# WhatAShot/Electrocardio-Panorama

Hardware: AMD Instinct MI355X
Metric: ECG-samples/sec (train step) (higher is better)
Workload: dtype f32 (conv products: fp32 operands split into fp16 hi+lo = 22-23 bits, block-scaled, 3 fp16 matrix products each, fp32 accumulate; fp32-class, not IEEE fp32)

## Files before the change

electrocardio_panorama_amd/_lib.py:

```python
import ctypes as C
import os

import torch

_HERE = os.path.dirname(os.path.abspath(__file__))
LIB_PATH = os.path.join(_HERE, "csrc", "libnefnet_hip.so")

NEF_OK = 0
_ERR = {-1: "NEF_E_SHAPE", -2: "NEF_E_NULL", -3: "NEF_E_WORKSPACE", -4: "NEF_E_UNSUPPORTED"}

p = C.c_void_p
i32 = C.c_int
i64 = C.c_int64
f32 = C.c_float
sz = C.c_size_t


class ConvArgs(C.Structure):
    _fields_ = [
        ("x", p), ("wp", p), ("y", p), ("bias", p), ("in_scale", p), ("res", p), ("gate", p), ("mask", p),
        ("x_bs", i64), ("x_gs", i64), ("y_bs", i64), ("y_gs", i64), ("sc_bs", i64), ("sc_gs", i64),
        ("res_bs", i64), ("res_gs", i64), ("gate_bs", i64), ("gate_gs", i64),
        ("B", i32), ("T", i32), ("G", i32), ("Cin_g", i32), ("Cout_g", i32), ("K", i32),
        ("relu", i32), ("gate_scale", f32), ("drop_scale", f32), ("drop_p", f32), ("rng_seed", C.c_uint64),
        ("pro_a", p), ("pro_b", p), ("pro_mode", i32), ("pro_Bp", i32), ("rng_seed_dev", p), ("wino", i32),
        ("stats", p),
        ("bnb_x", p), ("bnb_mean", p), ("bnb_invstd", p), ("bnb_a", p), ("bnb_b", p), ("bnb_slots", p), ("bnb_Bp", i32),
        ("bnb_up", i32), ("x_scale", f32), ("reserved0", i32), ("x_amax", p), ("x_amax_next", p), ("x_clamped", p),
        ("res_scale", p), ("rs_bs", i64), ("rs_gs", i64), ("gate_rowscale", p), ("gr_bs", i64), ("gr_gs", i64),
        ("stats_mode", i32), ("reserved1", i32),
    ]


class BwwArgs(C.Structure):
    _fields_ = [
        ("x", p), ("gy", p), ("gw", p), ("ws", p), ("in_scale", p), ("pro_a", p), ("pro_b", p),
        ("x_amax", p), ("gy_amax", p), ("x_amax_next", p), ("gy_amax_next", p), ("clamped", p), ("ws_bytes", sz),
        ("x_bs", i64), ("x_gs", i64), ("gy_bs", i64), ("gy_gs", i64), ("sc_bs", i64), ("sc_gs", i64),
        ("B", i32), ("T", i32), ("G", i32), ("Cin_g", i32), ("Cout_g", i32), ("K", i32),
        ("pro_mode", i32), ("pro_Bp", i32), ("form", i32), ("x_scale", f32), ("gy_scale", f32), ("reserved0", i32),
    ]


class BnBwdArgs(C.Structure):
    _fields_ = [
        ("g", p), ("gout", p), ("out", p), ("wout", p), ("x", p), ("mean", p), ("invstd", p), ("a", p), ("b", p),
        ("gx", p), ("ggamma", p), ("gbeta", p), ("gx_chan_sum", p), ("slots", p), ("ws", p), ("ws_bytes", sz),
        ("P", i32), ("Bp", i32), ("C", i32), ("L", i32), ("nslot", i32), ("form", i32), ("phase_major", i32), ("reserved0", i32),
    ]


class UpdateArgs(C.Structure):
    _fields_ = [
        ("p", p), ("g", p), ("buf", p), ("m", p), ("v", p), ("step", p), ("skip_if_positive", p), ("skipped", p), ("lr_dev", p),
        ("run_end", p), ("run_mul", p), ("n", i64), ("beta1", C.c_double), ("beta2", C.c_double),
        ("lr", f32), ("gscale", f32), ("mu", f32), ("eps", f32), ("weight_decay", f32),
        ("rule", i32), ("nesterov", i32), ("n_runs", i32),
    ]


class EmaArgs(C.Structure):
    _fields_ = [("ema", p), ("n_averaged", p), ("decay", C.c_double), ("warmup", i32), ("reserved0", i32)]


class PackDesc(C.Structure):
    _fields_ = [("w", p), ("wp", p), ("G", i32), ("Cog", i32), ("Cig", i32), ("K", i32), ("transpose_flip", i32),
                ("wino", i32), ("src_mode", i32), ("src_Cr", i32)]


SIGNATURES = {
    "nef_abi_version": (i32, []),
    "nef_debug_spin_us": (i32, [f32, i32, p]),
    "nef_stem_fwd": (i32, [p, p, p, i32, i32, i32, p]),
    "nef_stem_bwd_ws_bytes": (sz, [i32]),
    "nef_stem_bwd_weight": (i32, [p, p, p, p, p, sz, i32, i32, i32, p]),
    "nef_pack_weight": (i32, [p, p, i32, i32, i32, i32, i32, p]),
    "nef_pack_weight_wino": (i32, [p, p, i32, i32, i32, i32, i32, p]),
    "nef_pack_weight_wino4": (i32, [p, p, i32, i32, i32, i32, i32, p]),
    "nef_pack_weights": (i32, [C.POINTER(PackDesc), i32, p]),
    "nef_pack_weight_h2": (i32, [p, p, i32, i32, i32, i32, i32, p]),
    "nef_pack_weight_h2_bytes": (sz, [i32, i32, i32, i32, i32]),
    "nef_conv_fwd": (i32, [C.POINTER(ConvArgs), p]),
# ... 18 lines not shown
    "nef_theta_encode": (i32, [p, p, i32, p]),
    "nef_chscale_fwd": (i32, [p, p, i64, p, i32, i32, i32, p]),
    "nef_chscale_bwd": (i32, [p, p, p, i64, p, p, i32, i32, i32, i32, p]),
    "nef_gate": (i32, [p, p, p, f32, i64, p]),
    "nef_add": (i32, [p, p, p, i64, p]),
    "nef_roi_align_fwd": (i32, [p, p, p, i32, i32, i32, i32, i32, p]),
    "nef_roi_align_bwd": (i32, [p, p, p, i32, i32, i32, i32, i32, p]),
    "nef_window_crop": (i32, [p, i64, i64, p, i32, i32, i32, i32, i32, i32, p]),
    "nef_window_scatter": (i32, [p, p, i64, i64, i32, i32, i32, i32, i32, i32, p]),
    "nef_roi_unpool_fwd": (i32, [p, p, p, p, i32, i32, i32, p]),
    "nef_roi_unpool_bwd": (i32, [p, p, p, i32, i32, i32, p]),
    "nef_roi_segment_table": (i32, [p, p, p, i32, p]),
    "nef_lead_mean": (i32, [p, p, p, i32, i32, i32, p]),
    "nef_mix_fwd": (i32, [p, p, p, p, p, i32, i32, i32, i32, i32, p, p]),
    "nef_mix_bwd": (i32, [p, p, p, p, p, p, p, p, i32, i32, i32, i32, i32, p, i32, i32, i32, p]),
    "nef_mix_fwd_shared": (i32, [p, p, p, p, p, i32, i32, i32, i32, i32, p, p]),
    "nef_lead_mean_mix_shared": (i32, [p, p, p, p, p, i32, i32, i32, i32, i32, p, p]),
    "nef_pass_combine_fwd": (i32, [p, p, p, i32, i32, i32, p]),
    "nef_pass_combine_bwd": (i32, [p, p, i32, i32, i32, p]),
    "nef_pass_combine_stats_ws_bytes": (sz, [i32, i32]),
    "nef_pass_combine_fwd_stats": (i32, [p, p, p, p, p, p, p, p, p, p, p, p, sz, i32, i32, i32, f32, f32, p, p]),
    "nef_upsample2_fwd": (i32, [p, p, i64, i32, p]),
    "nef_upsample2_bwd": (i32, [p, p, i64, i32, p]),
    "nef_bn_ws_bytes": (sz, [i32, i32]),
    "nef_bn_train_stats": (i32, [p, p, p, p, p, p, p, p, p, p, sz, i32, i32, i32, i32, f32, f32, p, p]),
    "nef_conv_stats_slots": (i32, [i32, i32]),
    "nef_bn_stats_from_slots": (i32, [p, i32, p, p, p, p, p, p, p, p, p, sz, i32, i32, i32, i32, f32, f32, p, p]),
    "nef_bn_eval_affine": (i32, [p, p, p, p, p, p, i32, f32, p]),
    "nef_fold_bn": (i32, [p, p, p, p, p, p, i32, i32, p]),
    "nef_affine_relu_fwd": (i32, [p, p, p, p, i32, i32, i32, i32, p]),
    "nef_bn_bwd_ws_bytes": (sz, [C.POINTER(BnBwdArgs)]),
    "nef_bn_relu_bwd": (i32, [C.POINTER(BnBwdArgs), p]),
    "nef_bn_bwd_args_bytes": (sz, []),
    "nef_outconv_fwd": (i32, [p, p, p, i32, p, p, p, i32, i32, i32, p]),
    "nef_outconv_bwd_weight": (i32, [p, p, p, p, p, i32, p, p, p, sz, i32, i32, i32, p]),
    "nef_outconv_bwd_data": (i32, [p, p, p, p, i32, i32, i32, p]),
    "nef_outconv_bwd_weight_ws_bytes": (sz, [i32]),
    "nef_loss_ws_bytes": (sz, []),
    "nef_loss_fwd": (i32, [p, p, p, p, p, p, sz, i64, f32, f32, f32, i32, i32, p]),
    "nef_loss_bwd": (i32, [p, p, p, p, p, p, p, p, i64, f32, f32, f32, i32, i32, p]),
    "nef_loss_noise_fwd": (i32, [p, p, p, p, p, p, p, sz, i64, f32, f32, f32, i32, i32, p]),
    "nef_loss_noise_bwd": (i32, [p, p, p, p, p, p, p, p, p, i64, f32, f32, f32, i32, i32, p]),
    "nef_sgd_momentum": (i32, [p, p, p, i64, f32, f32, f32, i32, p, p, p, p]),
    "nef_adam": (i32, [p, p, p, p, i64, f32, C.c_double, C.c_double, f32, f32, f32, p, p, p, p, p]),
    "nef_update": (i32, [C.POINTER(UpdateArgs), p]),
    "nef_update_args_bytes": (sz, []),
    "nef_update_ema": (i32, [C.POINTER(UpdateArgs), C.POINTER(EmaArgs), p]),
    "nef_ema_args_bytes": (sz, []),
    "nef_grad_clip_ws_bytes": (sz, []),
    "nef_grad_clip": (i32, [p, i64, f32, f32, p, p, p, sz, p]),
    "nef_h2_taint": (i32, [p, p, p, p]),
    "nef_amax_roll": (i32, [p, p, i32, f32, f32, i32, p]),
    "nef_step_words": (i32, [p, p, i32, i32, i64, p]),
    "nef_flatten": (i32, [C.POINTER(p), C.POINTER(i64), i32, p, p]),
    "nef_regroup_halves": (i32, [p, p, i32, i32, i32, i32, p]),
    "nef_slots_to_rows": (i32, [p, i32, p, i32, i32, p]),
    "nef_poly_weights": (i32, [p, p, i32, i32, i32, p]),
    "nef_poly_fwd_edge": (i32, [p, p, p, i32, i32, i32, i32, i32, p, p, i32, p, i32, p, p]),
    "nef_poly_wgrad_fold_ws_bytes": (sz, [i32, i32, i32, i32]),
    "nef_poly_wgrad_fold": (i32, [p, p, p, p, p, sz, i32, i32, i32, i32, i32, p]),
    "nef_poly_bwd_edge": (i32, [p, p, p, i32, i32, i32, i32, i32, p, p, p, p, p, i32, p, i32, i32, p]),
    "nef_view_metrics": (i32, [p, p, p, p, p, i32, i32, i32, p]),
    "nef_pano_h_from_f32": (i32, [p, p, i32, i32, i32, p]),
    "nef_pano_h_pack_weight": (i32, [p, p, i32, i32, p]),
    "nef_pano_h_conv": (i32, [p, p, p, p, p, i32, i32, i32, i32, i32, i32, i32, i64, i64, p]),
    "nef_pano_h_conv_pair": (i32, [p, p, p, p, p, p, p, i32, i32, i32, i32, i64, i64, p]),
    "nef_pano_h_conv_outconv": (i32, [p, p, p, p, p, p, i32, i32, i32, i64, i64, p]),
    "nef_pano_h_conv_tail": (i32, [p, p, p, p, p, p, p, p, i32, i32, i32, i64, i64, p]),
    "nef_pano_h_outconv": (i32, [p, p, p, p, i32, i32, i32, i64, i64, p]),
}

_lib = None


class NefLibraryError(RuntimeError):
    pass


def load():
    global _lib
    if _lib is not None:
        return _lib
    if not os.path.exists(LIB_PATH):
        raise NefLibraryError(
            f"{LIB_PATH} not found: the HIP extension is required (no CPU fallback). "
            "Build it with `python -m electrocardio_panorama_amd.csrc.build`.")
    lib = C.CDLL(LIB_PATH)
    for name, (res, args) in SIGNATURES.items():
        fn = getattr(lib, name)
        fn.restype = res
        fn.argtypes = args
    for name, size, mirror in (("nef_conv_args", lib.nef_conv_args_bytes(), ConvArgs),
                               ("nef_bww_args", lib.nef_bww_args_bytes(), BwwArgs),
                               ("nef_bn_bwd_args", lib.nef_bn_bwd_args_bytes(), BnBwdArgs),
                               ("nef_update_args", lib.nef_update_args_bytes(), UpdateArgs),
                               ("nef_ema_args", lib.nef_ema_args_bytes(), EmaArgs)):
        if size != C.sizeof(mirror):
            raise NefLibraryError(f"{LIB_PATH}: {name} is {size} bytes, the binding mirrors {C.sizeof(mirror)}; rebuild with "
                                  "`python -m electrocardio_panorama_amd.csrc.build`")
    _lib = lib
    return lib


def check(rc, what=""):
    if rc == NEF_OK:
        return
    if rc < 0:
        raise NefLibraryError(f"{what}: {_ERR.get(rc, rc)}")
    raise NefLibraryError(f"{what}: hipError_t {rc}")
```

electrocardio_panorama_amd/csrc/elementwise.hip:

```cpp
#include "nef_common.h"

namespace {

__global__ void chscale_fwd_kernel(const float* __restrict__ x, const float* __restrict__ s, int64_t s_bs,
                                   float* __restrict__ y, int B, int C, int T) {
    const int64_t rows = (int64_t)B * C;
    const int wave = threadIdx.x >> 6, lane = threadIdx.x & 63;
    for (int64_t row = (int64_t)blockIdx.x * 4 + wave; row < rows; row += (int64_t)gridDim.x * 4) {
        const int b = (int)(row / C), c = (int)(row % C);
        const float f = s[(int64_t)b * s_bs + c];
        const float* xr = x + row * T;
        float* yr = y + row * T;
        for (int t = lane; t < T; t += 64) yr[t] = xr[t] * f;
    }
}

__global__ void chscale_bwd_kernel(const float* __restrict__ gy, const float* __restrict__ x,
                                   const float* __restrict__ s, int64_t s_bs, float* __restrict__ gx,
                                   float* __restrict__ gs, int B, int C, int T, int relu_x) {
    const int64_t rows = (int64_t)B * C;
    const int wave = threadIdx.x >> 6, lane = threadIdx.x & 63;
    for (int64_t row = (int64_t)blockIdx.x * 4 + wave; row < rows; row += (int64_t)gridDim.x * 4) {
        const int b = (int)(row / C), c = (int)(row % C);
        const float f = s[(int64_t)b * s_bs + c];
// ... 658 lines not shown
                s2 += (double)g * (double)((xv - mf) * is);
            }
        }
    }
    s1 = nef_block_sum_d(s1, sm);
    s2 = nef_block_sum_d(s2, sm);
    if (threadIdx.x == 0) {
        part[((int64_t)(p * C + c) * BN_SPLIT + sp) * 2] = s1;
        part[((int64_t)(p * C + c) * BN_SPLIT + sp) * 2 + 1] = s2;
    }
}

__global__ void bn_bwd_final(const double* __restrict__ part, float* __restrict__ coef, float* __restrict__ ggamma,
                             float* __restrict__ gbeta, int P, int Bp, int C, int L, int nsplit = BN_SPLIT) {
    const int c = blockIdx.x * blockDim.x + threadIdx.x;
    if (c >= C) return;
    const double n = (double)Bp * (double)L;
    double g1 = 0.0, g2 = 0.0;
    for (int p = 0; p < P; ++p) {
        double s1 = 0.0, s2 = 0.0;
        for (int sp = 0; sp < nsplit; ++sp) {
            s1 += part[((int64_t)(p * C + c) * nsplit + sp) * 2];
            s2 += part[((int64_t)(p * C + c) * nsplit + sp) * 2 + 1];
        }
        coef[(p * C + c) * 2] = (float)(s1 / n);
        coef[(p * C + c) * 2 + 1] = (float)(s2 / n);
        g1 += s1;
        g2 += s2;
    }
    gbeta[c] = (float)g1;
    ggamma[c] = (float)g2;
}

__global__ void bn_bwd_apply(const float* __restrict__ gy, const float* __restrict__ x, const float* __restrict__ mean,
                             const float* __restrict__ invstd, const float* __restrict__ a, const float* __restrict__ b,
                             const float* __restrict__ coef, float* __restrict__ gx, double* __restrict__ rowsum, int P,
                             int Bp, int C, int L) {
    const int64_t rows = (int64_t)P * Bp * C;
    const int wave = threadIdx.x >> 6, lane = threadIdx.x & 63;
    for (int64_t row = (int64_t)blockIdx.x * 4 + wave; row < rows; row += (int64_t)gridDim.x * 4) {
        const int c = (int)(row % C);
        const int p = (int)(row / ((int64_t)Bp * C));
        const int pc = p * C + c;
        const float mf = mean[pc], is = invstd[pc], af = a[pc], bf = b[pc];
        const float k1 = coef[pc * 2], k2 = coef[pc * 2 + 1];
        const float* xr = x + row * L;
        const float* gr = gy + row * L;
        float* gxr = gx + row * L;
        double rs = 0.0;
        if ((L & 3) == 0) {
            const int L4 = L >> 2;
#pragma unroll 2
            for (int t = lane; t < L4; t += 64) {
                const nef_f32x4 xv = ((const nef_f32x4*)xr)[t], gv = ((const nef_f32x4*)gr)[t];
                nef_f32x4 o;
#pragma unroll
                for (int e = 0; e < 4; ++e) {
                    const float g = fmaf(xv[e], af, bf) > 0.f ? gv[e] : 0.f;
                    o[e] = af * (g - k1 - (xv[e] - mf) * is * k2);
                    rs += (double)o[e];
                }
                ((nef_f32x4*)gxr)[t] = o;
            }
        } else {
            for (int t = lane; t < L; t += 64) {
                const float xv = xr[t];
// ... 1446 lines not shown
        if (form == 1)
            hipLaunchKernelGGL(bn_bwd_partial<1>, grid, dim3(256), 0, NEF_ST, g, a.x, a.mean, a.invstd, a.a, a.b, part, P, Bp, C, L,
                               a.wout);
        else if (form == 2)
            hipLaunchKernelGGL(bn_bwd_partial<2>, grid, dim3(256), 0, NEF_ST, g, a.x, a.mean, a.invstd, a.a, a.b, part, P, Bp, C, L,
                               (const float*)nullptr);
        else
            hipLaunchKernelGGL(bn_bwd_partial<0>, grid, dim3(256), 0, NEF_ST, g, a.x, a.mean, a.invstd, a.a, a.b, part, P, Bp, C, L,
                               (const float*)nullptr);
        hipLaunchKernelGGL(bn_bwd_final, dim3((C + 63) / 64), dim3(64), 0, NEF_ST, (const double*)part, coef, a.ggamma, a.gbeta, P, Bp, C,
                           L, BN_SPLIT);
    }
    const dim3 grid((unsigned)rows);
    if (form == 3)
        hipLaunchKernelGGL(bn_bwd_apply_combine3, dim3((unsigned)(Bp * C)), dim3(256), 0, NEF_ST, g, a.x, a.mean, a.invstd, a.a, a.b,
                           (const float*)coef, a.gx, rowsum, Bp, C, L, deint);
    else if (form == 2)
        hipLaunchKernelGGL(bn_bwd_apply_rows<2>, grid, dim3(256), 0, NEF_ST, g, a.x, a.mean, a.invstd, a.a, a.b, (const float*)coef, a.gx,
                           rowsum, Bp, C, L >> 2, (const float*)nullptr);
    else if (form == 1)
        hipLaunchKernelGGL(bn_bwd_apply_rows<1>, grid, dim3(256), 0, NEF_ST, g, a.x, a.mean, a.invstd, a.a, a.b, (const float*)coef, a.gx,
                           rowsum, Bp, C, L >> 2, a.wout);
    else if (by_rows)
        hipLaunchKernelGGL(bn_bwd_apply_rows<0>, grid, dim3(256), 0, NEF_ST, g, a.x, a.mean, a.invstd, a.a, a.b, (const float*)coef, a.gx,
                           rowsum, Bp, C, L >> 2, (const float*)nullptr, deint);
    else
        hipLaunchKernelGGL(bn_bwd_apply, dim3(nef_stream_grid(rows, 4)), dim3(256), 0, NEF_ST, g, a.x, a.mean, a.invstd, a.a, a.b,
                           (const float*)coef, a.gx, rowsum, P, Bp, C, L);
    if (a.gx_chan_sum)
        hipLaunchKernelGGL(rowsum_to_channel, dim3(C), dim3(256), 0, NEF_ST, (const double*)rowsum, a.gx_chan_sum, P * Bp, C);
    return nef_launch_status();
}

int nef_outconv_fwd(const float* x, const float* a, const float* b, int Bp, const float* w, const float* bias,
                    float* out, int N, int C, int L, nef_stream_t stream) {
    NEF_ENTER();
    NEF_REQUIRE(x && w && bias && out, NEF_E_NULL);
    NEF_REQUIRE((a == nullptr) == (b == nullptr), NEF_E_NULL);
    NEF_REQUIRE(N > 0 && C > 0 && C <= OC_MAXC && L > 0 && (!a || Bp > 0), NEF_E_SHAPE);
    if ((L & 3) == 0) {
        const int tiles = (L + 1023) / 1024;
        hipLaunchKernelGGL(outconv_fwd_kernel<true>, dim3((unsigned)((int64_t)N * tiles)), dim3(256), 0, NEF_ST, x, w, bias,
                           out, N, C, L, tiles, a, b, a ? Bp : 1);
        return nef_launch_status();
    }
    const int tiles = (L + 255) / 256;
    hipLaunchKernelGGL(outconv_fwd_kernel<false>, dim3((unsigned)((int64_t)N * tiles)), dim3(256), 0, NEF_ST, x, w, bias,
                       out, N, C, L, tiles, a, b, a ? Bp : 1);
    return nef_launch_status();
}

int nef_outconv_bwd_data(const float* gout, const float* out, const float* w, float* gx, int N, int C, int L,
                         nef_stream_t stream) {
    NEF_ENTER();
    NEF_REQUIRE(gout && out && w && gx, NEF_E_NULL);
    NEF_REQUIRE(N > 0 && C > 0 && C <= OC_MAXC && L > 0, NEF_E_SHAPE);
    const int tiles = (L + 255) / 256;
    hipLaunchKernelGGL(outconv_bwd_data_kernel, dim3((unsigned)((int64_t)N * tiles)), dim3(256), 0, NEF_ST, gout, out,
                       w, gx, N, C, L, tiles);
    return nef_launch_status();
}

size_t nef_outconv_bwd_weight_ws_bytes(int C) { return (size_t)OC_BLOCKS * (C + 1) * 3 * sizeof(double); }

int nef_outconv_bwd_weight(const float* gout, const float* out, const float* x, const float* a, const float* b, int Bp,
                           float* gw, float* gb, void* ws, size_t ws_bytes, int N, int C, int L, nef_stream_t stream) {
// ... 254 lines not shown
```

electrocardio_panorama_amd/engine.py:

```python
import os

import torch
from . import _env

from . import ops
from .ops import GV

N_SEG, ROI_BINS = 7, 16
DROP_P = 0.2
BN_EPS, BN_MOM = 1e-5, 0.1


DROPOUT_SITES = ("W_encoder.layer1.0", "W_encoder.layer1.1", "W_encoder.layer1.2", "w_conv.0", "z1_conv.0",
                 "z2_conv1.0", "z2_conv2.0", "z2_conv2.2")


class DropCfg:

    def __init__(self, training, p=DROP_P, masks=None, seed=0, seed_dev=None):
        self.seed_dev = seed_dev
        self.on = bool(training) and p > 0.0
        self.p = p if self.on else 0.0
        self.scale = 1.0 / (1.0 - p) if self.on else 1.0
        self.masks = masks
# ... 107 lines not shown
    xv, h, y, prefix, K, Cog, res_conv, dscale = saved[:8]
    in_scale = saved[8] if len(saved) > 8 else None
    side = side or ops._Inline()
    G, Cig = xv.G, xv.Cg
    g2 = gy if pre_gated else ops.gate(gy, y)
    g2v, hv = GV.dense(g2, G), GV.dense(h, G)
    grads[prefix + ".conv2.weight"] = side.run(lambda: ops.conv_bwd_weight(hv, g2v, K, site=P[prefix + ".conv2.weight"].data_ptr()), h, g2)
    gc1 = ops.conv(g2v, ops.pack_weight(P[prefix + ".conv2.weight"], G, flip=True, T=xv.T, f4=_bwd_f4(K)), Cog, K, gate=hv,
                   gate_scale=dscale, role="conv_bwd_data")
    gc1v = GV.dense(gc1, G)
    grads[prefix + ".conv1.weight"] = side.run(lambda: ops.conv_bwd_weight(xv, gc1v, K, in_scale=in_scale, site=P[prefix + ".conv1.weight"].data_ptr()), xv.t, gc1)
    if res_conv:
        grads[prefix + ".residual_conv.weight"] = side.run(lambda: ops.conv_bwd_weight(xv, g2v, 1, site=P[prefix + ".residual_conv.weight"].data_ptr()), xv.t, g2)
        grads[prefix + ".residual_conv.bias"] = side.run(lambda: ops.chan_sum(g2), g2)
        gres = ops.conv(g2v, ops.pack_weight(P[prefix + ".residual_conv.weight"], G, flip=True, T=xv.T), Cig, 1,
                        role="conv_bwd_data")
        resv = GV.dense(gres, G)
    else:
        resv = g2v
    wp1f = ops.pack_weight(P[prefix + ".conv1.weight"], G, flip=True, T=xv.T, f4=_bwd_f4(K))
    if in_scale is not None and scale_bwd and int(getattr(wp1f, "nef_wino", 0)) == 3 and out is None:
        slots = ops.conv_stats_buffer(wp1f, xv.B, G, Cig, xv.T, xv.t.device)
        if slots is not None:
            gx = ops.conv(gc1v, wp1f, Cig, K, res=resv, gate=xv, gate_scale=1.0, gate_rowscale=in_scale, stats=slots, stats_mode=1,
                          role="conv_bwd_data")
            return gx, ops.slots_to_rows(slots, xv.B)
    return ops.conv(gc1v, wp1f, Cig, K, res=resv,
                    out=out, gate=xv if gate_input else None, gate_scale=1.0, role="conv_bwd_data")


_DEC = (("decoder.1", "0", "1", 128), ("decoder.1", "3", "4", 128), ("decoder.3", "0", "1", 64),
        ("decoder.3", "3", "4", 64))


_HALVES = "decoder.1.double_conv.0.weight#halves"


def _regroup_halves(w, P=None):
    if P is not None:
        hit = P.get(_HALVES)
        if hit is not None and hit[1] is w and hit[2] == w._version:
            return hit[0]
    wg = ops.regroup_halves(w)
    if P is not None:
        P[_HALVES] = (wg, w, w._version)
    return wg


def _ungroup_halves(w2):
    return ops.regroup_halves(w2, inverse=True)


def _fusable(D, passes):
    return 2 * D.shape[2] >= 128


def _decoder_fwd_unfused(D, P, Bf, passes, training, save):
    x = D
    saved = []
    for li, (blk, cv, bn, cout) in enumerate(_DEC):
        if li in (0, 2):
            x = ops.upsample2_fwd(x)
        wname, bname, pre = f"{blk}.double_conv.{cv}.weight", f"{blk}.double_conv.{cv}.bias", f"{blk}.double_conv.{bn}"
        c = ops.conv(GV.dense(x, 1), ops.pack_weight(P[wname], 1, T=x.shape[2], f4=True), cout, 3, bias=P[bname])
        if training:
            mean, invstd, a, b = ops.bn_train_stats(c, P[pre + ".weight"], P[pre + ".bias"], Bf[pre + ".running_mean"],
# ... 56 lines not shown
        else:
            wp = ops.pack_weight(P[wname], 1, T=T_out, f4=True)
            slots = ops.conv_stats_buffer(wp, N, 1, cout, T_out, D.device) if training else None
            c = ops.conv(GV.dense(x_in, 1), wp, cout, 3, bias=P[bname], pro=pro, stats=slots)
            if slots is not None:
                stats = ops.bn_stats_from_slots(slots, P[pre + ".weight"], P[pre + ".bias"], Bf[pre + ".running_mean"],
                                                Bf[pre + ".running_var"], passes, N, T_out, BN_EPS, BN_MOM,
                                                nbt=Bf[pre + ".num_batches_tracked"])
        if stats is not None:
            mean, invstd, a, b = stats
            Bp = N // passes
        elif training:
            mean, invstd, a, b = ops.bn_train_stats(c, P[pre + ".weight"], P[pre + ".bias"], Bf[pre + ".running_mean"],
                                                    Bf[pre + ".running_var"], passes, BN_EPS, BN_MOM, nbt=Bf[pre + ".num_batches_tracked"])
            Bp = N // passes
        else:
            a, b = ops.bn_eval_affine(P[pre + ".weight"], P[pre + ".bias"], Bf[pre + ".running_mean"],
                                      Bf[pre + ".running_var"], BN_EPS)
            mean = invstd = None
            Bp = N
        if save:
            saved.append((x_in, c, mean, invstd, a, b, pro, up_after, xedge))
        x, pro_in = c, (a, b, Bp)
    out = ops.outconv_fwd(x, P["decoder.4.weight"], P["decoder.4.bias"], pro=pro_in)
    return out, (saved, x, out, passes, pro_in, shared_B)


def decoder_bwd(dsaved, g_out, P, grads, side=None):
    saved, c4, out, passes, pro4 = dsaved[:5]
    shared_B = dsaved[5] if len(dsaved) > 5 else None
    side = side or ops._Inline()
    if len(dsaved) > 5:
        ops.pack_many(_decoder_pack_requests(P, c4.shape[2] // 4, True))
    grads["decoder.4.weight"], grads["decoder.4.bias"] = side.run(
        lambda: ops.outconv_bwd_weight(g_out, out, c4, pro=pro4), g_out, out, c4)
    fuse_last = c4.shape[2] % 4 == 0
    g_is_up = False
    g = None if fuse_last else ops.outconv_bwd_data(g_out, out, P["decoder.4.weight"], c4.shape[1])
    g_slots = None
    poly_first = False
    for li in (3, 2, 1, 0):
        blk, cv, bn, cout = _DEC[li]
        x, c, mean, invstd, a, b, pro, up_after = saved[li][:8]
        xedge = saved[li][8] if len(saved[li]) > 8 else None
        sh0 = li == 0 and shared_B is not None
        Cog_, Cig_ = c.shape[1], x.shape[1] // (2 if sh0 else 1)
        poly_b = bool(up_after and pro[0] & 2 and (not sh0 or pro[0] == 2) and ops.poly_bwd_ok(2 if sh0 else 1, Cog_, Cig_, c.shape[2]))
        pm = bool(poly_b and xedge is not None and ops.poly_w_ok((2 if sh0 else 1) * (shared_B if sh0 else c.shape[0]), 2 if sh0 else 1, Cog_, Cig_, c.shape[2]))
        wname, bname, pre = f"{blk}.double_conv.{cv}.weight", f"{blk}.double_conv.{cv}.bias", f"{blk}.double_conv.{bn}"
        pm0_done = False
        if li == 3 and fuse_last:
            gc, gg, gbeta, gbias = ops.bn_relu_bwd_outconv(g_out, out, P["decoder.4.weight"], c, mean, invstd, a, b, passes)
        elif li == 0 and shared_B is not None and not g_is_up:
            gc, gg, gbeta, gbias = ops.bn_relu_bwd_combine3(g, c, mean, invstd, a, b, slots=g_slots, phase_major=pm)
            pm0_done = pm
        elif g_is_up:
            gc, gg, gbeta, gbias = ops.bn_relu_bwd_up(g, c, mean, invstd, a, b, passes, slots=g_slots)
        else:
            gc, gg, gbeta, gbias = ops.bn_relu_bwd(g, c, P[pre + ".weight"], mean, invstd, a, b, passes,
                                                   with_chan_sum=True, slots=g_slots, phase_major=pm and not sh0)
            pm0_done = pm and not sh0
        grads[pre + ".weight"], grads[pre + ".bias"], grads[bname] = gg, gbeta, gbias
        pm = pm and pm0_done
        if li == 0 and shared_B is not None:
            gp2 = gc if gc.shape[0] == 2 * shared_B else ops.pass_combine_bwd(gc)
            gpv, xv = GV.dense(gp2, 2), GV.dense(x, 2)
            if pm:
                grads[wname] = side.run(lambda: _ungroup_halves(ops.conv_bwd_weight_poly(xv, gp2, Cog_, pro, xedge, site=P[wname].data_ptr())), x, gp2, xedge)
            else:
                grads[wname] = side.run(lambda: _ungroup_halves(ops.conv_bwd_weight(xv, gpv, 3, pro=pro, site=P[wname].data_ptr())), x, gp2)
            if poly_b:
                g = ops.conv_bwd_data_poly(gpv, _regroup_halves(P[wname], P), x.shape[1] // 2, site=P[wname].data_ptr(), phase_major=pm)
                poly_first = True
            else:
                g = ops.conv(gpv, ops.pack_weight(_regroup_halves(P[wname], P), 2, flip=True, T=gp2.shape[2], f4=True, site=P[wname].data_ptr()), x.shape[1] // 2, 3,
                             role="conv_bwd_data")
        else:
            gcv, xv = GV.dense(gc, 1), GV.dense(x, 1)
            if pm:
                grads[wname] = side.run(lambda: ops.conv_bwd_weight_poly(xv, gc, Cog_, pro, xedge, site=P[wname].data_ptr()), x, gc, xedge)
            else:
                grads[wname] = side.run(lambda: ops.conv_bwd_weight(xv, gcv, 3, pro=pro, site=P[wname].data_ptr()), x, gc)
            if poly_b:
                bnb = None
# ... 324 lines not shown
```

electrocardio_panorama_amd/ops.py:

```python
import ctypes as C
import contextlib
import itertools
import os

import torch
from . import _env

from . import _lib

N_SEG, ROI_BINS = 7, 16


def _p(t):
    return None if t is None else t.data_ptr()


def _stream():
    return torch.cuda.current_stream().cuda_stream


def _chk(t, dtype=torch.float32):
    assert t.is_cuda and t.dtype == dtype and t.is_contiguous(), (t.device, t.dtype, t.is_contiguous())
    return t

# ... 1249 lines not shown

def bn_relu_bwd(gy, x, gamma, mean, invstd, a, b, P, with_chan_sum=False, slots=None, phase_major=False):
    _chk(gy), _chk(x)
    N, Ct, Ln = x.shape
    gx = torch.empty(N, 2 * Ct, Ln // 2, device=x.device, dtype=torch.float32) if phase_major else torch.empty_like(x)
    r = _bn_bwd(0, "bn_relu_bwd", (gy, x, gx), x, mean, invstd, a, b, P, gx, with_chan_sum, slots, phase_major, g=gy)
    return r if with_chan_sum else r[:3]


def bn_relu_bwd_combine3(gy, x, mean, invstd, a, b, slots=None, phase_major=False):
    _chk(gy), _chk(x)
    N, Ct, Ln = x.shape
    Bp = N // 3
    gP2 = torch.empty((2 * Bp, 4 * Ct, Ln // 2) if phase_major else (2 * Bp, 2 * Ct, Ln), device=x.device, dtype=torch.float32)
    return _bn_bwd(3, "bn_relu_bwd_combine3", (gy, x, gP2), x, mean, invstd, a, b, 3, gP2, slots=slots, phase_major=phase_major,
                   g=gy)


def bn_relu_bwd_up(gu, x, mean, invstd, a, b, P, slots=None):
    _chk(gu), _chk(x)
    N, Ct, Ln = x.shape
    assert gu.shape == (N, Ct, 2 * Ln)
    gx = torch.empty_like(x)
    return _bn_bwd(2, "bn_relu_bwd_up", (gu, x, gx), x, mean, invstd, a, b, P, gx, slots=slots, g=gu)


def bn_relu_bwd_outconv(gout, out, wout, x, mean, invstd, a, b, P):
    _chk(gout), _chk(out), _chk(x)
    gx = torch.empty_like(x)
    return _bn_bwd(1, "bn_relu_bwd_outconv", (gout, out, x, gout, out, x, gx), x, mean, invstd, a, b, P, gx, gout=gout, out=out,
                   wout=wout)


def outconv_fwd(x, w, bias, pro=None):
    L = _lib.load()
    _chk(x), _chk(w), _chk(bias)
    N, Ct, Ln = x.shape
    out = torch.empty(N, 1, Ln, device=x.device, dtype=torch.float32)
    a, b, Bp = pro if pro is not None else (None, None, 1)
    ev = _hbm("outconv_fwd", x, out)
    _lib.check(L.nef_outconv_fwd(_p(x), _p(a), _p(b), Bp, _p(w), _p(bias), _p(out), N, Ct, Ln, _stream()), "nef_outconv_fwd")
    _done(ev)
    return out


def outconv_bwd_data(gout, out, w, Ct):
    L = _lib.load()
    _chk(gout), _chk(out)
    N, Ln = out.shape[0], out.shape[-1]
    gx = torch.empty(N, Ct, Ln, device=out.device, dtype=torch.float32)
    _lib.check(L.nef_outconv_bwd_data(_p(gout), _p(out), _p(w), _p(gx), N, Ct, Ln, _stream()), "nef_outconv_bwd_data")
    return gx


def outconv_bwd_weight(gout, out, x, pro=None):
    L = _lib.load()
    _chk(gout), _chk(out), _chk(x)
    N, Ct, Ln = x.shape
    gw = torch.empty(1, Ct, 3, device=x.device, dtype=torch.float32)
    gb = torch.empty(1, device=x.device, dtype=torch.float32)
    n = L.nef_outconv_bwd_weight_ws_bytes(Ct)
    ws = workspace(n, x.device)
    a, b, Bp = pro if pro is not None else (None, None, 1)
    ev = _hbm("outconv_bwd_weight", gout, out, x)
    _lib.check(L.nef_outconv_bwd_weight(_p(gout), _p(out), _p(x), _p(a), _p(b), Bp, _p(gw), _p(gb), _p(ws), n, N, Ct, Ln,
                                        _stream()), "nef_outconv_bwd_weight")
# ... 258 lines not shown
```

include/nefnet_hip.h:

```cpp
#ifndef NEFNET_HIP_H
#define NEFNET_HIP_H

#include <stddef.h>
#include <stdint.h>

#ifdef __cplusplus
extern "C" {
#endif

#define NEF_OK 0
#define NEF_E_SHAPE (-1)
#define NEF_E_NULL (-2)
#define NEF_E_WORKSPACE (-3)
#define NEF_E_UNSUPPORTED (-4)

#define NEF_N_SEG 7
#define NEF_ROI_BINS 16

typedef void* nef_stream_t;

int nef_abi_version(void);

int nef_debug_spin_us(float us, int wgs, nef_stream_t stream);

// ... 187 lines not shown
                       float* a, float* b, int C, float eps, nef_stream_t stream);
int nef_fold_bn(const float* w, const float* bias, const float* a, const float* b, float* w_out, float* bias_out,
                int Cout, int inner, nef_stream_t stream);
int nef_affine_relu_fwd(const float* x, const float* a, const float* b, float* y, int P, int Bp, int C, int L,
                        nef_stream_t stream);
typedef struct nef_bn_bwd_args {
    const float* g;
    const float* gout;
    const float* out;
    const float* wout;
    const float* x;
    const float* mean;
    const float* invstd;
    const float* a;
    const float* b;
    float* gx;
    float* ggamma;
    float* gbeta;
    float* gx_chan_sum;
    const float* slots;
    void* ws;
    size_t ws_bytes;
    int32_t P, Bp, C, L;
    int32_t nslot;
    int32_t form;
    int32_t phase_major;
    int32_t reserved0;
} nef_bn_bwd_args;

int nef_bn_relu_bwd(const nef_bn_bwd_args* a, nef_stream_t stream);
size_t nef_bn_bwd_ws_bytes(const nef_bn_bwd_args* a);
size_t nef_bn_bwd_args_bytes(void);

int nef_outconv_fwd(const float* x, const float* a, const float* b, int Bp, const float* w, const float* bias,
                    float* out, int N, int C, int L, nef_stream_t stream);
int nef_outconv_bwd_weight(const float* gout, const float* out, const float* x, const float* a, const float* b, int Bp,
                           float* gw, float* gb, void* ws, size_t ws_bytes, int N, int C, int L, nef_stream_t stream);
int nef_outconv_bwd_data(const float* gout, const float* out, const float* w, float* gx, int N, int C, int L,
                         nef_stream_t stream);
size_t nef_outconv_bwd_weight_ws_bytes(int C);

size_t nef_loss_ws_bytes(void);
int nef_loss_fwd(const float* pred, const float* pred_p, const float* pred_l, const float* target, float* losses,
                 void* ws, size_t ws_bytes, int64_t n, float f0, float f1, float f2, int reg_l2, int use_mask,
                 nef_stream_t stream);
int nef_loss_bwd(const float* pred, const float* pred_p, const float* pred_l, const float* target,
                 const float* gscale , float* g_pred, float* g_p, float* g_l, int64_t n, float f0,
                 float f1, float f2, int reg_l2, int use_mask, nef_stream_t stream);
int nef_loss_noise_fwd(const float* pred, const float* pred_p, const float* pred_l, const float* target,
                       const float* noise, float* losses, void* ws, size_t ws_bytes, int64_t n, float f0, float f1, float f2,
                       int reg_l2, int use_mask, nef_stream_t stream);
int nef_loss_noise_bwd(const float* pred, const float* pred_p, const float* pred_l, const float* target,
                       const float* noise, const float* gscale , float* g_pred, float* g_p, float* g_l,
                       int64_t n, float f0, float f1, float f2, int reg_l2, int use_mask, nef_stream_t stream);

int nef_sgd_momentum(float* p, const float* g, float* buf, int64_t n, float lr, float mu, float gscale,
                     int first_step, const float* skip_if_positive , int32_t* skipped , const float* lr_dev , nef_stream_t stream);
int nef_adam(float* p, const float* g, float* m, float* v, int64_t n, float lr, double beta1, double beta2, float eps,
             float weight_decay, float gscale, float* step , const float* skip_if_positive,
             int32_t* skipped, const float* lr_dev, nef_stream_t stream);
#define NEF_UPDATE_MAX_RUNS 256
typedef struct nef_update_args {
    float* p;
    const float* g;
    float* buf;
    float* m;
// ... 76 lines not shown
```

Measured before the change: 8624.

## Fuse output-conv weight gradient into last BN-ReLU backward reduction pass

After: 8659 (median of 6 runs). About the same (+0.4%).

```diff
diff --git a/electrocardio_panorama_amd/_lib.py b/electrocardio_panorama_amd/_lib.py
--- a/electrocardio_panorama_amd/_lib.py
+++ b/electrocardio_panorama_amd/_lib.py
@@ -48,6 +48,10 @@
         ("gx", p), ("ggamma", p), ("gbeta", p), ("gx_chan_sum", p), ("slots", p), ("ws", p), ("ws_bytes", sz),
         ("P", i32), ("Bp", i32), ("C", i32), ("L", i32), ("nslot", i32), ("form", i32), ("phase_major", i32), ("reserved0", i32),
     ]
+
+
+class LastBnArgs(C.Structure):
+    _fields_ = [("go", p), ("coef", p), ("gwout", p), ("gbout", p), ("gbias", p)]
 
 
 class UpdateArgs(C.Structure):
@@ -132,6 +136,9 @@
     "nef_bn_bwd_ws_bytes": (sz, [C.POINTER(BnBwdArgs)]),
     "nef_bn_relu_bwd": (i32, [C.POINTER(BnBwdArgs), p]),
     "nef_bn_bwd_args_bytes": (sz, []),
+    "nef_lastbn_bwd": (i32, [C.POINTER(BnBwdArgs), C.POINTER(LastBnArgs), p]),
+    "nef_lastbn_bwd_ws_bytes": (sz, [C.POINTER(BnBwdArgs)]),
+    "nef_lastbn_args_bytes": (sz, []),
     "nef_outconv_fwd": (i32, [p, p, p, i32, p, p, p, i32, i32, i32, p]),
     "nef_outconv_bwd_weight": (i32, [p, p, p, p, p, i32, p, p, p, sz, i32, i32, i32, p]),
     "nef_outconv_bwd_data": (i32, [p, p, p, p, i32, i32, i32, p]),
@@ -193,6 +200,7 @@
     for name, size, mirror in (("nef_conv_args", lib.nef_conv_args_bytes(), ConvArgs),
                                ("nef_bww_args", lib.nef_bww_args_bytes(), BwwArgs),
                                ("nef_bn_bwd_args", lib.nef_bn_bwd_args_bytes(), BnBwdArgs),
+                               ("nef_lastbn_args", lib.nef_lastbn_args_bytes(), LastBnArgs),
                                ("nef_update_args", lib.nef_update_args_bytes(), UpdateArgs),
                                ("nef_ema_args", lib.nef_ema_args_bytes(), EmaArgs)):
         if size != C.sizeof(mirror):
diff --git a/electrocardio_panorama_amd/csrc/elementwise.hip b/electrocardio_panorama_amd/csrc/elementwise.hip
--- a/electrocardio_panorama_amd/csrc/elementwise.hip
+++ b/electrocardio_panorama_amd/csrc/elementwise.hip
@@ -714,6 +714,104 @@
     ggamma[c] = (float)g2;
 }
 
+constexpr int LB_NPART = 8;
+constexpr int LB_NU = 5;
+
+__global__ __launch_bounds__(256) void lastbn_sums_partial(const float* __restrict__ go, const float* __restrict__ x,
+                                                           const float* __restrict__ mean, const float* __restrict__ invstd,
+                                                           const float* __restrict__ a, const float* __restrict__ b,
+                                                           double* __restrict__ part, int P, int Bp, int C, int L,
+                                                           const float* __restrict__ ocw) {
+    __shared__ double sm[4];
+    int bid = blockIdx.x;
+    const int sp = bid % BN_SPLIT;
+    bid /= BN_SPLIT;
+    const int c = bid % C;
+    const int p = bid / C;
+    const float mf = mean[p * C + c], is = invstd[p * C + c], af = a[p * C + c], bf = b[p * C + c];
+    const float w0 = ocw[c * 3], w1 = ocw[c * 3 + 1], w2 = ocw[c * 3 + 2];
+    double s1 = 0.0, s2 = 0.0, sx = 0.0, gw0 = 0.0, gw1 = 0.0, gw2 = 0.0, gs = 0.0;
+    const int L4 = L >> 2;
+    for (int bb = sp; bb < Bp; bb += BN_SPLIT) {
+        const int64_t off = (((int64_t)p * Bp + bb) * C + c) * L;
+        const nef_f32x4* xr = (const nef_f32x4*)(x + off);
+        const float* gor = go + ((int64_t)p * Bp + bb) * L;
+        for (int tc = 0; tc < L4; tc += LB_NU * 256) {
+            nef_f32x4 xq[LB_NU];
+#pragma unroll
+            for (int u = 0; u < LB_NU; ++u) {
+                const int t = tc + u * 256 + threadIdx.x;
+                if (t < L4) xq[u] = xr[t];
+            }
+#pragma unroll
+            for (int u = 0; u < LB_NU; ++u) {
+                const int t = tc + u * 256 + threadIdx.x;
+                if (t >= L4) continue;
+                const nef_f32x4 xv = xq[u], gv = oc_grad4(gor, t, L, w0, w1, w2);
+                const nef_f32x4 m = *(const nef_f32x4*)(gor + 4 * t);
+                const double gd[6] = {(double)(t > 0 ? gor[4 * t - 1] : 0.f), (double)m[0], (double)m[1], (double)m[2], (double)m[3],
+                                      (double)(4 * t + 4 < L ? gor[4 * t + 4] : 0.f)};
+#pragma unroll
+                for (int e = 0; e < 4; ++e) {
+                    const float y = fmaf(xv[e], af, bf);
+                    const float g = y > 0.f ? gv[e] : 0.f;
+                    const float xh = (xv[e] - mf) * is;
+                    s1 += (double)g;
+                    s2 += (double)g * (double)xh;
+                    sx += (double)xh;
+                    const double v = (double)fmaxf(y, 0.f);
+                    gw0 = fma(gd[e + 2], v, gw0);
+                    gw1 = fma(gd[e + 1], v, gw1);
+                    gw2 = fma(gd[e], v, gw2);
+                }
+                if (c == 0) gs += (gd[1] + gd[2]) + (gd[3] + gd[4]);
+            }
+        }
+    }
+    double r[7] = {s1, s2, sx, gw0, gw1, gw2, gs};
+#pragma unroll
+    for (int i = 0; i < 7; ++i) r[i] = nef_block_sum_d(r[i], sm);
+    if (threadIdx.x == 0) {
+        double* o = part + ((int64_t)(p * C + c) * BN_SPLIT + sp) * LB_NPART;
+#pragma unroll
+        for (int i = 0; i < 7; ++i) o[i] = r[i];
+    }
+}
+
+__global__ void lastbn_final(const double* __restrict__ part, const float* __restrict__ a, float* __restrict__ coef,
+                             float* __restrict__ ggamma, float* __restrict__ gbeta, float* __restrict__ gwout,
+                             float* __restrict__ gbout, float* __restrict__ gbias, int P, int Bp, int C, int L) {
+    const int c = blockIdx.x * blockDim.x + threadIdx.x;
+    if (c >= C) return;
+    const double n = (double)Bp * (double)L;
+    double g1 = 0.0, g2 = 0.0, gw[3] = {0.0, 0.0, 0.0}, gs = 0.0, gbi = 0.0;
+    for (int p = 0; p < P; ++p) {
+        double s1 = 0.0, s2 = 0.0, sx = 0.0;
+        for (int sp = 0; sp < BN_SPLIT; ++sp) {
+            const double* q = part + ((int64_t)(p * C + c) * BN_SPLIT + sp) * LB_NPART;
+            s1 += q[0];
+            s2 += q[1];
+            sx += q[2];
+            gw[0] += q[3];
+            gw[1] += q[4];
+            gw[2] += q[5];
+            gs += q[6];
+        }
+        const float k1 = (float)(s1 / n), k2 = (float)(s2 / n);
+        coef[(p * C + c) * 2] = k1;
+        coef[(p * C + c) * 2 + 1] = k2;
+        g1 += s1;
+        g2 += s2;
+        gbi += (double)a[p * C + c] * (s1 - n * (double)k1 - (double)k2 * sx);
+    }
+    gbeta[c] = (float)g1;
+    ggamma[c] = (float)g2;
+    gbias[c] = (float)gbi;
+#pragma unroll
+    for (int k = 0; k < 3; ++k) gwout[c * 3 + k] = (float)gw[k];
+    if (c == 0) gbout[0] = (float)gs;
+}
+
 __global__ void bn_bwd_apply(const float* __restrict__ gy, const float* __restrict__ x, const float* __restrict__ mean,
                              const float* __restrict__ invstd, const float* __restrict__ a, const float* __restrict__ b,
                              const float* __restrict__ coef, float* __restrict__ gx, double* __restrict__ rowsum, int P,
@@ -2226,6 +2324,37 @@
     return nef_launch_status();
 }
 
+size_t nef_lastbn_args_bytes(void) { return sizeof(nef_lastbn_args); }
+
+size_t nef_lastbn_bwd_ws_bytes(const nef_bn_bwd_args* a) {
+    if (!a || a->form != 1 || a->P <= 0 || a->Bp <= 0 || a->C <= 0 || a->L <= 0) return 0;
+    return (size_t)a->P * a->C * BN_SPLIT * LB_NPART * sizeof(double);
+}
+
+int nef_lastbn_bwd(const nef_bn_bwd_args* args, const nef_lastbn_args* last, nef_stream_t stream) {
+    NEF_ENTER();
+    NEF_REQUIRE(args && last, NEF_E_NULL);
+    const nef_bn_bwd_args& a = *args;
+    const int P = a.P, Bp = a.Bp, C = a.C, L = a.L;
+    NEF_REQUIRE(a.x && a.mean && a.invstd && a.a && a.b && a.ggamma && a.gbeta && a.ws && a.gout && a.out && a.wout, NEF_E_NULL);
+    NEF_REQUIRE(last->go && last->coef && last->gwout && last->gbout && last->gbias, NEF_E_NULL);
+    NEF_REQUIRE(a.form == 1 && !a.g && !a.slots && !a.phase_major && !a.gx_chan_sum, NEF_E_UNSUPPORTED);
+    NEF_REQUIRE(P > 0 && Bp > 0 && C > 0 && L > 0, NEF_E_SHAPE);
+    const int64_t rows = (int64_t)P * Bp * C;
+    NEF_REQUIRE((L & 3) == 0 && rows <= 0x7FFFFFFF && (int64_t)P * C * BN_SPLIT <= 0x7FFFFFFF, NEF_E_SHAPE);
+    NEF_REQUIRE(a.ws_bytes >= nef_lastbn_bwd_ws_bytes(args), NEF_E_WORKSPACE);
+    const int64_t n = (int64_t)P * Bp * L;
+    hipLaunchKernelGGL(outconv_go_kernel, dim3(nef_stream_grid(n, 256)), dim3(256), 0, NEF_ST, a.gout, a.out, last->go, n);
+    hipLaunchKernelGGL(lastbn_sums_partial, dim3(P * C * BN_SPLIT), dim3(256), 0, NEF_ST, (const float*)last->go, a.x, a.mean, a.invstd,
+                       a.a, a.b, (double*)a.ws, P, Bp, C, L, a.wout);
+    hipLaunchKernelGGL(lastbn_final, dim3((C + 63) / 64), dim3(64), 0, NEF_ST, (const double*)a.ws, a.a, last->coef, a.ggamma, a.gbeta,
+                       last->gwout, last->gbout, last->gbias, P, Bp, C, L);
+    if (a.gx)
+        hipLaunchKernelGGL(bn_bwd_apply_rows<1>, dim3((unsigned)rows), dim3(256), 0, NEF_ST, (const float*)last->go, a.x, a.mean,
+                           a.invstd, a.a, a.b, (const float*)last->coef, a.gx, (double*)nullptr, Bp, C, L >> 2, a.wout);
+    return nef_launch_status();
+}
+
 int nef_outconv_fwd(const float* x, const float* a, const float* b, int Bp, const float* w, const float* bias,
                     float* out, int N, int C, int L, nef_stream_t stream) {
     NEF_ENTER();
diff --git a/electrocardio_panorama_amd/engine.py b/electrocardio_panorama_amd/engine.py
--- a/electrocardio_panorama_amd/engine.py
+++ b/electrocardio_panorama_amd/engine.py
@@ -163,6 +163,8 @@
 _DEC = (("decoder.1", "0", "1", 128), ("decoder.1", "3", "4", 128), ("decoder.3", "0", "1", 64),
         ("decoder.3", "3", "4", 64))
 
+
+LASTBN_SUMS = True
 
 _HALVES = "decoder.1.double_conv.0.weight#halves"
 
@@ -285,9 +287,11 @@
     side = side or ops._Inline()
     if len(dsaved) > 5:
         ops.pack_many(_decoder_pack_requests(P, c4.shape[2] // 4, True))
-    grads["decoder.4.weight"], grads["decoder.4.bias"] = side.run(
-        lambda: ops.outconv_bwd_weight(g_out, out, c4, pro=pro4), g_out, out, c4)
     fuse_last = c4.shape[2] % 4 == 0
+    last_sums = bool(LASTBN_SUMS and fuse_last and pro4 is not None and saved[3][2] is not None and c4 is saved[3][1])
+    if not last_sums:
+        grads["decoder.4.weight"], grads["decoder.4.bias"] = side.run(
+            lambda: ops.outconv_bwd_weight(g_out, out, c4, pro=pro4), g_out, out, c4)
     g_is_up = False
     g = None if fuse_last else ops.outconv_bwd_data(g_out, out, P["decoder.4.weight"], c4.shape[1])
     g_slots = None
@@ -302,7 +306,10 @@
         pm = bool(poly_b and xedge is not None and ops.poly_w_ok((2 if sh0 else 1) * (shared_B if sh0 else c.shape[0]), 2 if sh0 else 1, Cog_, Cig_, c.shape[2]))
         wname, bname, pre = f"{blk}.double_conv.{cv}.weight", f"{blk}.double_conv.{cv}.bias", f"{blk}.double_conv.{bn}"
         pm0_done = False
-        if li == 3 and fuse_last:
+        if li == 3 and last_sums:
+            gc, gg, gbeta, gbias, grads["decoder.4.weight"], grads["decoder.4.bias"] = ops.lastbn_bwd(
+                g_out, out, P["decoder.4.weight"], c, mean, invstd, a, b, passes)[:6]
+        elif li == 3 and fuse_last:
             gc, gg, gbeta, gbias = ops.bn_relu_bwd_outconv(g_out, out, P["decoder.4.weight"], c, mean, invstd, a, b, passes)
         elif li == 0 and shared_B is not None and not g_is_up:
             gc, gg, gbeta, gbias = ops.bn_relu_bwd_combine3(g, c, mean, invstd, a, b, slots=g_slots, phase_major=pm)
diff --git a/electrocardio_panorama_amd/ops.py b/electrocardio_panorama_amd/ops.py
--- a/electrocardio_panorama_amd/ops.py
+++ b/electrocardio_panorama_amd/ops.py
@@ -1305,6 +1305,28 @@
                    wout=wout)
 
 
+def lastbn_bwd(gout, out, wout, x, mean, invstd, a, b, P, apply=True):
+    L = _lib.load()
+    _chk(gout), _chk(out), _chk(x)
+    N, Ct, Ln = x.shape
+    dev = x.device
+    gx = torch.empty_like(x) if apply else None
+    gg, gb, gs = (torch.empty(Ct, device=dev, dtype=torch.float32) for _ in range(3))
+    go = torch.empty(N, Ln, device=dev, dtype=torch.float32)
+    coef = torch.empty(P, Ct, 2, device=dev, dtype=torch.float32)
+    gw = torch.empty(1, Ct, 3, device=dev, dtype=torch.float32)
+    gbo = torch.empty(1, device=dev, dtype=torch.float32)
+    A = _lib.BnBwdArgs(x=_p(x), mean=_p(mean), invstd=_p(invstd), a=_p(a), b=_p(b), gx=_p(gx), ggamma=_p(gg), gbeta=_p(gb),
+                       gout=_p(gout), out=_p(out), wout=_p(wout), P=P, Bp=N // P, C=Ct, L=Ln, form=1)
+    B_ = _lib.LastBnArgs(go=_p(go), coef=_p(coef), gwout=_p(gw), gbout=_p(gbo), gbias=_p(gs))
+    A.ws_bytes = L.nef_lastbn_bwd_ws_bytes(C.byref(A))
+    A.ws = _p(workspace(A.ws_bytes, dev))
+    ev = _hbm("lastbn_bwd", gout, out, go, x, go, *((go, x, gx) if apply else ()))
+    _lib.check(L.nef_lastbn_bwd(C.byref(A), C.byref(B_), _stream()), "nef_lastbn_bwd")
+    _done(ev)
+    return gx, gg, gb, gs, gw, gbo, go, coef
+
+
 def outconv_fwd(x, w, bias, pro=None):
     L = _lib.load()
     _chk(x), _chk(w), _chk(bias)
diff --git a/include/nefnet_hip.h b/include/nefnet_hip.h
--- a/include/nefnet_hip.h
+++ b/include/nefnet_hip.h
@@ -243,6 +243,18 @@
 size_t nef_bn_bwd_ws_bytes(const nef_bn_bwd_args* a);
 size_t nef_bn_bwd_args_bytes(void);
 
+typedef struct nef_lastbn_args {
+    float* go;
+    float* coef;
+    float* gwout;
+    float* gbout;
+    float* gbias;
+} nef_lastbn_args;
+
+int nef_lastbn_bwd(const nef_bn_bwd_args* a, const nef_lastbn_args* last, nef_stream_t stream);
+size_t nef_lastbn_bwd_ws_bytes(const nef_bn_bwd_args* a);
+size_t nef_lastbn_args_bytes(void);
+
 int nef_outconv_fwd(const float* x, const float* a, const float* b, int Bp, const float* w, const float* bias,
                     float* out, int N, int C, int L, nef_stream_t stream);
 int nef_outconv_bwd_weight(const float* gout, const float* out, const float* x, const float* a, const float* b, int Bp,
```
